# yangzhaojason/DualDiff

Measured on AMD Instinct MI355X. Metric: denoising-steps/sec, 6-view 224×400 fp16, 50-step DDIM @ 1/2/4/8 MI355X, higher is better.
Workload: dtype fp16; 1 GPU; BASELINE configs[1]: 6-view 224x400 (28x50 latents) multiview UNet + 2 ControlNet branches (ORS panorama + ORS-3D, SFA on), CFG 2.0 -> 12 view-instances/scene, DDIM-50 schedule, random-init weights; scenes_per_gpu=1, parallelism=scene-sharded x1 (no data-path collective), hip_graph=True, streams=3, invariant_conditioning=recomputed every step

## Files before the change

### dualdiff_amd/_native.py

```python
import ctypes
import os

import torch
from ctypes import (POINTER, Structure, c_char_p, c_float, c_int32, c_int64, c_uint32, c_void_p)

from . import _build

DD_F16, DD_BF16, DD_F32 = 0, 1, 2
DD_EPI_NONE, DD_EPI_GEGLU, DD_EPI_SILU = 0, 1, 2


class GemmDesc(Structure):
    _fields_ = [
        ("a", c_void_p), ("a2", c_void_p), ("lda", c_int64), ("lda2", c_int64), ("k1", c_int32),
        ("rows", c_int32), ("n", c_int32), ("k", c_int32),
        ("w", c_void_p), ("bias", c_void_p), ("rowvec", c_void_p),
        ("rows_per_inst", c_int32), ("ld_rowvec", c_int32),
        ("res", c_void_p), ("ldres", c_int64),
        ("out", c_void_p), ("ldc", c_int64),
        ("alpha", c_float), ("accumulate", c_int32), ("epilogue", c_int32),
        ("conv", c_int32), ("hin", c_int32), ("win", c_int32), ("cin", c_int32),
        ("hv", c_int32), ("wv", c_int32), ("hout", c_int32), ("wout", c_int32), ("stride", c_int32),
        ("dtype", c_int32), ("tile", c_int32), ("split_k", c_int32),
        ("ws", c_void_p), ("ws_bytes", c_int64),
# ... 28 lines not shown
        ("pos", c_void_p), ("cat", c_void_p), ("cls_out", c_void_p),
        ("rows", c_int32), ("points_per_box", c_int32), ("num_freqs", c_int32), ("include_input", c_int32),
        ("class_token_dim", c_int32), ("cls_offset", c_int32),
        ("ld_cat", c_int64),
        ("normalize", c_int32), ("points_dtype", c_int32), ("dtype", c_int32), ("n_classes", c_int32),
        ("freqs", c_float * 16), ("xyz_min", c_float * 3), ("xyz_range", c_float * 3),
    ]


class XAttnDesc(Structure):
    _fields_ = [
        ("x", c_void_p), ("ldx", c_int64), ("res", c_void_p), ("ldres", c_int64),
        ("wq", c_void_p), ("wo", c_void_p), ("bo", c_void_p),
        ("k", c_void_p), ("v", c_void_p), ("ldk", c_int64), ("ldv", c_int64),
        ("k_inst_stride", c_int64), ("k_head_stride", c_int64), ("v_inst_stride", c_int64), ("v_head_stride", c_int64),
        ("out", c_void_p), ("ldo", c_int64),
        ("instances", c_int32), ("rows_per_inst", c_int32), ("lk", c_int32),
        ("channels", c_int32), ("heads", c_int32), ("scale", c_float), ("dtype", c_int32),
        ("ln_out", c_void_p), ("ld_ln_out", c_int64), ("ln_gamma", c_void_p), ("ln_beta", c_void_p), ("ln_eps", c_float),
        ("lk_dev", c_void_p),
    ]


class Gemm8Desc(Structure):
    _fields_ = [
        ("a", c_void_p), ("a_scale", c_void_p), ("lda", c_int64),
        ("w", c_void_p), ("w_scale", c_void_p), ("ldw", c_int64),
        ("bias", c_void_p), ("res", c_void_p), ("ldres", c_int64),
        ("out", c_void_p), ("ldc", c_int64),
        ("rows", c_int32), ("n", c_int32), ("k_padded", c_int32), ("dtype", c_int32),
        ("out_headmajor_d", c_int32), ("hm_scaled_planes", c_int32), ("hm_scale", c_float), ("geglu", c_int32),
    ]


SIGNATURES = {
    "dd_abi_version": (c_int32, []),
    "dd_desc_size": (c_int64, [c_int32]),
    "dd_error_string": (c_char_p, [c_int32]),
    "dd_target_arch": (c_char_p, []),
    "dd_gemm": (c_int32, [POINTER(GemmDesc), c_void_p]),
    "dd_gemm_workspace_bytes": (c_int64, [POINTER(GemmDesc)]),
    "dd_gemm_num_tiles": (c_int32, []),
    "dd_gemm_tile_id": (c_int32, [c_int32]),
    "dd_gemm_kernel_name": (c_char_p, [POINTER(GemmDesc)]),
    "dd_gemm_conv_pad": (c_int32, [POINTER(GemmDesc), c_int32, c_void_p]),
    "dd_gemm_conv_pad_workspace_bytes": (c_int64, [POINTER(GemmDesc), c_int32]),
    "dd_gemm_conv_pad_kernel_name": (c_char_p, [POINTER(GemmDesc), c_int32]),
    "dd_groupnorm_nhwc": (c_int32, [c_void_p, c_int32, c_void_p, c_int32, c_void_p, c_void_p, c_void_p,
                                    c_int32, c_int32, c_int32, c_float, c_int32, c_int32,
                                    c_void_p, c_int64, c_void_p]),
    "dd_groupnorm_workspace_bytes": (c_int64, [c_int32, c_int32]),
    "dd_groupnorm_is_fused": (c_int32, [c_int32, c_int32, c_int32]),
    "dd_layernorm": (c_int32, [c_void_p, c_void_p, c_void_p, c_void_p, c_int64, c_int32, c_float,
                               c_int32, c_void_p]),
    "dd_attention": (c_int32, [POINTER(AttnDesc), c_void_p]),
    "dd_attention_kernel_name": (c_char_p, [POINTER(AttnDesc)]),
    "dd_add": (c_int32, [c_void_p, c_void_p, c_void_p, c_void_p, c_int64, c_int32, c_void_p]),
    "dd_scale": (c_int32, [c_void_p, c_void_p, c_float, c_int64, c_int32, c_void_p]),
    "dd_probe_spin": (c_int32, [c_void_p, c_uint32, c_void_p]),
    "dd_groupnorm_splitk": (c_int32, [c_void_p, c_int32, c_void_p, c_void_p, c_int32, c_void_p, c_int64, c_void_p,
                                      c_void_p, c_void_p, c_void_p, c_int32, c_int32, c_int32, c_int32, c_float, c_int32,
                                      c_int32, c_void_p]),
    "dd_xattn320": (c_int32, [POINTER(XAttnDesc), c_void_p]),
    "dd_nchw_to_nhwc_views": (c_int32, [c_void_p, c_void_p, c_int32, c_int32, c_int32, c_int32, c_int32, c_int32, c_int32,
                                        c_void_p]),
    "dd_fourier_embed_strided": (c_int32, [c_void_p, c_void_p, c_int64, c_int32, POINTER(c_float), c_int32, c_int32,
                                           c_int32, c_int32, c_int32, c_int64, c_int64, c_int64, c_int64, c_void_p]),
    "dd_box_tokens": (c_int32, [POINTER(BoxTokensDesc), c_void_p]),
    "dd_ctx_assemble": (c_int32, [c_void_p, c_void_p, c_void_p, c_void_p, c_void_p, c_int32, c_int32, c_int32, c_int32,
                                  c_int32, c_int32, c_int32, c_int32, c_void_p]),
    "dd_gemm8": (c_int32, [POINTER(Gemm8Desc), c_void_p]),
    "dd_rowquant_fp8": (c_int32, [c_void_p, c_void_p, c_void_p, c_void_p, c_void_p, c_int64, c_int32, c_int64, c_float,
                                  c_int32, c_void_p]),
    "dd_xattn_pack_weight": (c_int32, [c_void_p, c_void_p, c_int32, c_void_p]),
    "dd_silu": (c_int32, [c_void_p, c_void_p, c_int64, c_int32, c_void_p]),
    "dd_nchw_to_nhwc": (c_int32, [c_void_p, c_void_p, c_int32, c_int32, c_int32, c_int32, c_int32, c_void_p]),
    "dd_nhwc_to_nchw": (c_int32, [c_void_p, c_void_p, c_int32, c_int32, c_int32, c_int32, c_int32, c_void_p]),
    "dd_timestep_embedding": (c_int32, [c_void_p, c_void_p, c_int32, c_int32, c_int32, c_float,
                                        c_int32, c_void_p]),
    "dd_cfg_unipc_step": (c_int32, [c_void_p, c_void_p, c_void_p, c_void_p, c_void_p, c_void_p, c_void_p, c_void_p,
                                    c_float, c_int64, c_int32, c_void_p]),
    "dd_softmax_rows": (c_int32, [c_void_p, c_void_p, c_int64, c_int32, c_int64, c_int64, c_int32, c_void_p]),
    "dd_ors_project": (c_int32, [c_void_p, c_void_p, c_void_p, c_void_p, c_void_p, c_int32, c_int32, c_int32,
                                 c_float, c_int32, c_int32, c_int32, c_void_p]),
    "dd_fourier_embed": (c_int32, [c_void_p, c_void_p, c_int64, c_int32, POINTER(c_float), c_int32, c_int32,
                                   c_int32, c_int32, c_void_p]),
    "dd_conv3x3_small_cout": (c_int32, [c_void_p, c_void_p, c_void_p, c_void_p, c_int32, c_int32,
                                        c_int32, c_int32, c_int32, c_int32, c_void_p]),
    "dd_vae_posterior": (c_int32, [c_void_p, c_void_p, c_void_p, c_void_p, c_void_p, c_int32, c_int32, c_int32, c_float,
                                   c_int32, c_int32, c_void_p]),
# ... 70 lines not shown
```

### dualdiff_amd/csrc/elementwise.hip

```cpp
#include "dd_common.h"

namespace {

template <typename T>
__global__ __launch_bounds__(256)
void dd_add_kernel(const T* a, const T* b, const T* c, T* y, int64_t nvec) {
  for (int64_t i = (int64_t)blockIdx.x * blockDim.x + threadIdx.x; i < nvec;
       i += (int64_t)gridDim.x * blockDim.x) {
    float fa[8], fb[8];
    dd_unpack8<T>(dd_ld16(a + i * 8), fa);
    dd_unpack8<T>(dd_ld16(b + i * 8), fb);
#pragma unroll
    for (int e = 0; e < 8; ++e) fa[e] += fb[e];
    if (c) {
      dd_unpack8<T>(dd_ld16(c + i * 8), fb);
#pragma unroll
      for (int e = 0; e < 8; ++e) fa[e] += fb[e];
    }
    dd_st16(y + i * 8, dd_pack8<T>(fa));
  }
}

template <typename T, int OP>
__global__ __launch_bounds__(256)
void dd_unary_kernel(const T* x, T* y, float s, int64_t nvec) {
  for (int64_t i = (int64_t)blockIdx.x * blockDim.x + threadIdx.x; i < nvec;
       i += (int64_t)gridDim.x * blockDim.x) {
    float f[8];
    dd_unpack8<T>(dd_ld16(x + i * 8), f);
#pragma unroll
    for (int e = 0; e < 8; ++e) f[e] = OP == 0 ? f[e] * s : dd_silu_f(f[e]);
    dd_st16(y + i * 8, dd_pack8<T>(f));
  }
}

template <typename T>
__global__ __launch_bounds__(256)
void dd_nchw_to_nhwc_kernel(const T* x, T* y, int m, int c, int hw, int c_pad) {
  const int64_t total = (int64_t)m * hw * c_pad;
  for (int64_t i = (int64_t)blockIdx.x * blockDim.x + threadIdx.x; i < total;
       i += (int64_t)gridDim.x * blockDim.x) {
    const int ch = (int)(i % c_pad);
    const int64_t row = i / c_pad;
    const int px = (int)(row % hw);
    const int inst = (int)(row / hw);
    y[i] = ch < c ? x[((int64_t)inst * c + ch) * hw + px] : (T)0.f;
  }
}

template <typename T>
__global__ __launch_bounds__(256)
void dd_nhwc_to_nchw_kernel(const T* x, T* y, int m, int c, int hw, int ldx) {
// ... 207 lines not shown
  T* yout = y + (int64_t)inst * hout * wout * COUT;
#pragma unroll
  for (int rr = 0; rr < ROWS_PER_WAVE; ++rr) {
    const int oy = oy0 + wave * ROWS_PER_WAVE + rr;
    if (oy >= hout) continue;
    const int prow = (wave * ROWS_PER_WAVE + rr) * STRIDE;
#pragma unroll
    for (int g = 0; g < TW / 16; ++g) {
      const int ox = ox0 + g * 16 + px;
      if (ox0 + g * 16 >= wout) continue;
      const unsigned char* base = smem + (size_t)(prow * PW + (g * 16 + px) * STRIDE) * PIX;
      f32x4 acc[NB];
#pragma unroll
      for (int nb = 0; nb < NB; ++nb) acc[nb] = f32x4{0.f, 0.f, 0.f, 0.f};
#pragma unroll
      for (int ks = 0; ks < KSTEPS; ++ks) {
        const V8 xf = dd_as_v8<T>(*reinterpret_cast<const u32x4*>(base + koff[ks]));
#pragma unroll
        for (int nb = 0; nb < NB; ++nb) acc[nb] = dd_mfma16(wf[nb][ks], xf, acc[nb]);
      }
      if (ox < wout) {
#pragma unroll
        for (int nb = 0; nb < NB; ++nb) {
          V4 o;
#pragma unroll
          for (int r = 0; r < 4; ++r) {
            float v = acc[nb][r] + bv[nb][r];
            if (silu) v = dd_silu_f(v);
            o[r] = (T)v;
          }
          *reinterpret_cast<V4*>(yout + ((int64_t)oy * wout + ox) * COUT + nb * 16 + kc * 4) = o;
        }
      }
    }
  }
}

template <typename T>
__device__ __forceinline__ float dd_cfg_guided(const T* eps, int64_t i, int64_t n, float guidance) {
  const float eu = (float)eps[i], ec = (float)eps[n + i];
  return (float)(T)(eu + guidance * (ec - eu));
}

struct dd_ddim_coef {
  float sa_t, s1a_t, sa_p, s1a_p;
  __device__ explicit dd_ddim_coef(const float* c) : sa_t(c[0]), s1a_t(c[1]), sa_p(c[2]), s1a_p(c[3]) {}
  __device__ __forceinline__ float step(float xv, float e) const {
    const float x0 = (xv - s1a_t * e) / sa_t;
    return sa_p * x0 + s1a_p * e;
  }
  __device__ __forceinline__ float step(float xv, float e, float*, float*, float*, int64_t) const { return step(xv, e); }
};

struct dd_unipc_coef {
  float a_x, a_e, use_c, c_l, c_1, c_2, c_0, p_x, p_0, p_1;
  __device__ explicit dd_unipc_coef(const float* c)
      : a_x(c[0]), a_e(c[1]), use_c(c[2]), c_l(c[3]), c_1(c[4]), c_2(c[5]), c_0(c[6]), p_x(c[7]), p_0(c[8]),
        p_1(c[9]) {}
  __device__ __forceinline__ float step(float xv, float e, float* last, float* m1, float* m2, int64_t i) const {
    const float x0 = a_x * xv + a_e * e;
    const float o1 = m1[i];
    float xc = xv;
    if (use_c != 0.f) xc = c_l * last[i] + c_1 * o1 + c_2 * m2[i] + c_0 * x0;
    const float r = p_x * xc + p_0 * x0 + p_1 * o1;
    last[i] = xc;
    m2[i] = o1;
// ... 89 lines not shown
  for (int j = blockIdx.x * blockDim.x + threadIdx.x; j < view_elems; j += gridDim.x * blockDim.x) {
    const T r = dd_add_noise<T>(sa, s1a, clean[base + j], noise0[base + j]);
    x[base + j] = r;
    if (x_dup) x_dup[base + j] = r;
  }
}

inline unsigned grid_for(int64_t work, int per_block = 256, unsigned cap = 2048) {
  int64_t b = (work + per_block - 1) / per_block;
  if (b > cap) b = cap;
  if (b < 1) b = 1;
  return (unsigned)b;
}

}

extern "C" int dd_add(const void* a, const void* b, const void* c, void* y, int64_t n,
                      int32_t dtype, dd_stream_t stream) {
  if (!a || !b || !y || n <= 0 || (n & 7)) return DD_ERR_BAD_ARG;
  if (dtype != DD_F16 && dtype != DD_BF16) return DD_ERR_BAD_ARG;
  if (!dd_aligned16(a) || !dd_aligned16(b) || !dd_aligned16(y) || (c && !dd_aligned16(c))) return DD_ERR_BAD_ARG;
  hipStream_t s = reinterpret_cast<hipStream_t>(stream);
  dd_clear_error();
  const int64_t nvec = n / 8;
  if (dtype == DD_F16)
    hipLaunchKernelGGL(dd_add_kernel<_Float16>, dim3(grid_for(nvec)), dim3(256), 0, s,
                       (const _Float16*)a, (const _Float16*)b, (const _Float16*)c, (_Float16*)y, nvec);
  else
    hipLaunchKernelGGL(dd_add_kernel<__bf16>, dim3(grid_for(nvec)), dim3(256), 0, s,
                       (const __bf16*)a, (const __bf16*)b, (const __bf16*)c, (__bf16*)y, nvec);
  return dd_check_launch();
}

extern "C" int dd_scale(const void* x, void* y, float sc, int64_t n, int32_t dtype, dd_stream_t stream) {
  if (!x || !y || n <= 0 || (n & 7)) return DD_ERR_BAD_ARG;
  if (dtype != DD_F16 && dtype != DD_BF16) return DD_ERR_BAD_ARG;
  if (!dd_aligned16(x) || !dd_aligned16(y)) return DD_ERR_BAD_ARG;
  hipStream_t s = reinterpret_cast<hipStream_t>(stream);
  dd_clear_error();
  const int64_t nvec = n / 8;
  if (dtype == DD_F16)
    hipLaunchKernelGGL((dd_unary_kernel<_Float16, 0>), dim3(grid_for(nvec)), dim3(256), 0, s,
                       (const _Float16*)x, (_Float16*)y, sc, nvec);
  else
    hipLaunchKernelGGL((dd_unary_kernel<__bf16, 0>), dim3(grid_for(nvec)), dim3(256), 0, s,
                       (const __bf16*)x, (__bf16*)y, sc, nvec);
  return dd_check_launch();
}

extern "C" int dd_silu(const void* x, void* y, int64_t n, int32_t dtype, dd_stream_t stream) {
  if (!x || !y || n <= 0 || (n & 7)) return DD_ERR_BAD_ARG;
  if (dtype != DD_F16 && dtype != DD_BF16) return DD_ERR_BAD_ARG;
  if (!dd_aligned16(x) || !dd_aligned16(y)) return DD_ERR_BAD_ARG;
  hipStream_t s = reinterpret_cast<hipStream_t>(stream);
  dd_clear_error();
  const int64_t nvec = n / 8;
  if (dtype == DD_F16)
    hipLaunchKernelGGL((dd_unary_kernel<_Float16, 1>), dim3(grid_for(nvec)), dim3(256), 0, s,
                       (const _Float16*)x, (_Float16*)y, 1.f, nvec);
  else
    hipLaunchKernelGGL((dd_unary_kernel<__bf16, 1>), dim3(grid_for(nvec)), dim3(256), 0, s,
                       (const __bf16*)x, (__bf16*)y, 1.f, nvec);
  return dd_check_launch();
}

extern "C" int dd_nchw_to_nhwc(const void* x, void* y, int32_t m, int32_t c, int32_t hw,
// ... 77 lines not shown
  return dd_check_launch();
}

template <typename TI>
int launch_fourier(const void* x, void* out, int64_t total, int dims, const FourierFreqs& fr, int nf, int inc,
                   int out_dtype, hipStream_t s) {
  const unsigned g = (unsigned)grid_for(total > (1 << 30) ? (1 << 30) : (int)total);
  if (out_dtype == DD_F16)
    hipLaunchKernelGGL((dd_fourier_embed_kernel<TI, _Float16>), dim3(g), dim3(256), 0, s, (const TI*)x, (_Float16*)out, total, dims, fr, nf, inc);
  else if (out_dtype == DD_BF16)
    hipLaunchKernelGGL((dd_fourier_embed_kernel<TI, __bf16>), dim3(g), dim3(256), 0, s, (const TI*)x, (__bf16*)out, total, dims, fr, nf, inc);
  else
    hipLaunchKernelGGL((dd_fourier_embed_kernel<TI, float>), dim3(g), dim3(256), 0, s, (const TI*)x, (float*)out, total, dims, fr, nf, inc);
  return dd_check_launch();
}

extern "C" int dd_fourier_embed(const void* x, void* out, int64_t rows, int32_t dims, const float* freqs,
                                int32_t num_freqs, int32_t include_input, int32_t in_dtype, int32_t out_dtype,
                                dd_stream_t stream) {
  if (!x || !out || !freqs || rows <= 0 || dims <= 0) return DD_ERR_BAD_ARG;
  if (num_freqs <= 0 || num_freqs > 16) return DD_ERR_UNSUPPORTED;
  if (in_dtype < 0 || in_dtype > DD_F32 || out_dtype < 0 || out_dtype > DD_F32) return DD_ERR_BAD_ARG;
  FourierFreqs fr{};
  for (int i = 0; i < num_freqs; ++i) fr.f[i] = freqs[i];
  hipStream_t s = reinterpret_cast<hipStream_t>(stream);
  dd_clear_error();
  const int64_t total = rows * dims;
  const int inc = include_input ? 1 : 0;
  if (in_dtype == DD_F16) return launch_fourier<_Float16>(x, out, total, dims, fr, num_freqs, inc, out_dtype, s);
  if (in_dtype == DD_BF16) return launch_fourier<__bf16>(x, out, total, dims, fr, num_freqs, inc, out_dtype, s);
  return launch_fourier<float>(x, out, total, dims, fr, num_freqs, inc, out_dtype, s);
}

extern "C" int dd_conv3x3_small_cout(const void* x, const void* w, const void* bias, void* y_nchw,
                                     int32_t m, int32_t h, int32_t wd, int32_t cin, int32_t cout,
                                     int32_t dtype, dd_stream_t stream) {
  if (!x || !w || !y_nchw || m <= 0 || h <= 0 || wd <= 0 || cin <= 0 || cout <= 0) return DD_ERR_BAD_ARG;
  if ((cin & 7) || cout > 8) return DD_ERR_UNSUPPORTED;
  if (dtype != DD_F16 && dtype != DD_BF16) return DD_ERR_BAD_ARG;
  if (!dd_aligned16(x) || !dd_aligned16(w)) return DD_ERR_BAD_ARG;
  hipStream_t s = reinterpret_cast<hipStream_t>(stream);
  dd_clear_error();
  const int64_t npix = (int64_t)m * h * wd;
  const unsigned blocks = (unsigned)((npix + 3) / 4);
  if (dtype == DD_F16)
    hipLaunchKernelGGL((dd_conv3x3_small_kernel<_Float16, 8>), dim3(blocks), dim3(256), 0, s,
                       (const _Float16*)x, (const _Float16*)w, (const _Float16*)bias,
                       (_Float16*)y_nchw, m, h, wd, cin, cout);
  else
    hipLaunchKernelGGL((dd_conv3x3_small_kernel<__bf16, 8>), dim3(blocks), dim3(256), 0, s,
                       (const __bf16*)x, (const __bf16*)w, (const __bf16*)bias,
                       (__bf16*)y_nchw, m, h, wd, cin, cout);
  return dd_check_launch();
}

template <typename T, int CIN, int COUT, int STRIDE>
static int launch_thin(const void* x, const void* w, const void* bias, void* y, int m, int hin, int win, int hout, int wout,
                       int silu, hipStream_t s) {
  constexpr int TW = 64, TH = STRIDE == 1 ? 8 : 4;
  constexpr int PW = (TW - 1) * STRIDE + 3, PH = (TH - 1) * STRIDE + 3;
  constexpr int PIX = CIN * 2 + (CIN > 8 ? 16 : 0);
  constexpr size_t smem = (size_t)PH * PW * PIX;
  static_assert(smem <= 64 * 1024, "patch fits the default dynamic LDS limit");
  dim3 grid(((wout + TW - 1) / TW) * ((hout + TH - 1) / TH), m);
  hipLaunchKernelGGL((dd_conv3x3_thin_kernel<T, CIN, COUT, STRIDE>), grid, dim3(256), smem, s, (const T*)x, (const T*)w,
                     (const T*)bias, (T*)y, hin, win, hout, wout, silu);
  return dd_check_launch();
}

template <typename T>
static int launch_thin_t(const void* x, const void* w, const void* bias, void* y, int m, int hin, int win, int hout, int wout,
                         int cin, int cout, int stride, int silu, hipStream_t s) {
#define DD_THIN(CI, CO, ST) if (cin == CI && cout == CO && stride == ST) \
    return launch_thin<T, CI, CO, ST>(x, w, bias, y, m, hin, win, hout, wout, silu, s);
  DD_THIN(8, 16, 1) DD_THIN(16, 16, 1) DD_THIN(16, 32, 2) DD_THIN(32, 32, 1)
// ... 181 lines not shown
```

### dualdiff_amd/networks/unet_2d_condition_multiview.py

```python
from dataclasses import dataclass
from typing import Any, Dict, Optional, Tuple, Union

import torch
import torch.nn as nn

from .. import ops as O
from .blocks import BasicMultiviewTransformerBlock
from .layers import (BasicTransformerBlock, prefetch_cross_kv, drop_prefetched_kv, CrossKVBank, Conv3x3, CrossAttnDownBlock2D, CrossAttnUpBlock2D, DownBlock2D, GroupNorm,
                     TimestepEmbedding, Timesteps, UNetMidBlock2DCrossAttn, UpBlock2D, as_nchw_view,
                     run_down_block, run_up_block, to_nhwc, CTX_BASE, context_keys, ctx_capacity, lk_const)
from .model_base import ModelBase, sibling_overlap


def _at_capacity(ctx, cap):
    m, lc, c = ctx.shape
    if lc == cap:
        return ctx
    if ctx.stride(2) == 1 and ctx.stride(1) == c and ctx.stride(0) == cap * c and \
            (ctx.storage_offset() + m * cap * c) * ctx.element_size() <= ctx.untyped_storage().nbytes():
        return ctx.as_strided((m, cap, c), ctx.stride())
    buf = ctx.new_zeros((m, cap, c))
    buf[:, :lc] = ctx
    return buf


@dataclass
class UNet2DConditionOutput:
    sample: torch.Tensor


_DEFAULT_PAIR = {0: [5, 1], 1: [0, 2], 2: [1, 3], 3: [2, 4], 4: [3, 5], 5: [4, 0]}


class UNet2DConditionModelMultiview(ModelBase):
    multiview = True
    video = False
    prefetch_kv = __import__('os').environ.get('DD_PREFETCH_KV', '0') == '1'
    kv_bank = __import__('os').environ.get('DD_KV_BANK', '1') != '0'

    _WARN_ONCE = 0

    def __init__(
        self,
        sample_size: Optional[int] = None,
        in_channels: int = 4,
        out_channels: int = 4,
        center_input_sample: bool = False,
        flip_sin_to_cos: bool = True,
        freq_shift: int = 0,
        down_block_types: Tuple[str] = ("CrossAttnDownBlock2D", "CrossAttnDownBlock2D",
                                        "CrossAttnDownBlock2D", "DownBlock2D"),
        mid_block_type: Optional[str] = "UNetMidBlock2DCrossAttn",
        up_block_types: Tuple[str] = ("UpBlock2D", "CrossAttnUpBlock2D", "CrossAttnUpBlock2D",
                                      "CrossAttnUpBlock2D"),
        only_cross_attention: Union[bool, Tuple[bool]] = False,
        block_out_channels: Tuple[int] = (320, 640, 1280, 1280),
# ... 184 lines not shown
        with context_keys(ctx2d, lc, lk_dev):
            return [self.forward_nhwc(x, m, h, w, t_f32, ctx2d, lc, down_res, mid_res)]

    def forward_nhwc(self, x, m, h, w, t_f32, ctx2d, lc, down_res=None, mid_res=None):
        state = self.encode_nhwc(x, m, h, w, t_f32, ctx2d, lc)
        return self.decode_nhwc(state, down_res, mid_res)

    def encode_nhwc(self, x, m, h, w, t_f32, ctx2d, lc):
        dt = self.dtype
        if self.kv_bank:
            if self.__dict__.get("_kv_bank") is None:
                self.__dict__["_kv_bank"] = CrossKVBank(self)
            self.__dict__["_kv_bank"].run(ctx2d)
        elif self.prefetch_kv:
            if self.__dict__.get("_kv_stream") is None:
                self.__dict__["_kv_stream"] = torch.cuda.Stream()
            prefetch_cross_kv(self, ctx2d, self.__dict__["_kv_stream"])
        emb = self.time_embedding.run(self.time_proj.run(t_f32, dt))
        temb = self.temb_bank.run(O.silu(emb))
        forward_size = any(s % (2 ** self.num_upsamplers) != 0 for s in (h, w))
        x = self.conv_in.run(x, m, h, w)
        skips = [(x, h, w)]
        for blk in self.down_blocks:
            x, h, w, s = run_down_block(blk, x, m, h, w, temb, ctx2d, lc)
            skips += s
        x = self.mid_block.run(x, m, h, w, temb, ctx2d, lc)
        return {"x": x, "m": m, "h": h, "w": w, "skips": skips, "temb": temb, "ctx2d": ctx2d, "lc": lc,
                "forward_size": forward_size}

    def decode_nhwc(self, state, down_res=None, mid_res=None):
        x, m, h, w = state["x"], state["m"], state["h"], state["w"]
        skips, temb, ctx2d, lc = list(state["skips"]), state["temb"], state["ctx2d"], state["lc"]

        def plus(t, r):
            if not isinstance(r, (tuple, list)):
                r = (r,)
            if len(r) == 0:
                return t
            i = 0
            while i < len(r):
                t = O.add(t, r[i], r[i + 1]) if i + 1 < len(r) else O.add(t, r[i])
                i += 2
            return t

        if down_res is not None:
            if len(down_res) != len(skips):
                raise ValueError("expected %d down-block residuals, got %d" % (len(skips), len(down_res)))
            skips = [(plus(s, r), sh, sw) for (s, sh, sw), r in zip(skips, down_res)]
        if mid_res is not None:
            x = plus(x, mid_res)
        for i, blk in enumerate(self.up_blocks):
            final = i == len(self.up_blocks) - 1
            k = len(blk.resnets)
            up_size = None
            if not final:
                nxt = skips[-k - 1]
                up_size = (nxt[1], nxt[2]) if state["forward_size"] else None
            x, h, w = run_up_block(blk, x, m, h, w, skips, temb, ctx2d, lc, up_size)
        a = self.conv_norm_out.run(x, m, h * w, True)
        if self.__dict__.get("_kv_stream") is not None:
            drop_prefetched_kv(self, self.__dict__["_kv_stream"])
        if self.__dict__.get("_kv_bank") is not None:
            self.__dict__["_kv_bank"].drop()
        return O.conv3x3_small_cout(a, self.conv_out.packed, self.conv_out.bias, m, h, w)



class UNet2DConditionModel(UNet2DConditionModelMultiview):
    multiview = False



class UNet2DConditionModelMultiviewVideo(UNet2DConditionModelMultiview):
    video = True

    def set_n_frames(self, n_frames):
        from .video_blocks import VideoMultiviewTransformerBlock
        for mod in self.modules():
            if isinstance(mod, VideoMultiviewTransformerBlock):
                mod.n_frames = int(n_frames)
        self.config["n_frames"] = int(n_frames)

    def set_frame_shard(self, shard):
# ... 9 lines not shown
```

### dualdiff_amd/ops.py

```python
import collections as _collections
import ctypes
import os as _os

import torch

from . import _native, _timer, _workspace, tuning
from ._native import DD_BF16, DD_EPI_GEGLU, DD_EPI_NONE, DD_EPI_SILU, DD_F16, AttnDesc, Gemm8Desc, GemmDesc, XAttnDesc
from ._timer import KernelTimer, _stream, set_timer
from ._workspace import workspace, workspace_owner
from .tuning import (CHALLENGE_TILES, TUNE_TABLE_PATH, forget_tuned, load_tuned, save_tuned,
                     tune_candidates, tuned_table)

_THIN_CONV = _os.environ.get("DD_THIN_CONV", "1") != "0"
GN_SPLITK = _os.environ.get("DD_GN_SPLITK", "0") == "1"
LN_OUT_TILE = int(_os.environ.get("DD_LN_OUT_TILE", "0"))
XATTN_MAX_WGS = int(_os.environ.get("DD_XATTN_MAX_WGS", "256"))
CAUSAL_ATTN_MAX_L = 128
_ZERO_BIAS = {}
_FDT = {torch.float16: 0, torch.bfloat16: 1, torch.float32: 2}


def _dtype_code(dtype):
    if dtype == torch.float16:
        return DD_F16
    if dtype == torch.bfloat16:
        return DD_BF16
    raise TypeError("dualdiff_amd ops take fp16 / bf16 tensors, got %s" % dtype)


def _dt(t):
    return _dtype_code(t.dtype)


def _tname(code):
    return "f16" if code == DD_F16 else "bf16"


def _need_gpu(*ts):
    for t in ts:
        if t is not None and not t.is_cuda:
# ... 478 lines not shown
        bo = _ZERO_BIAS[key]
    d.bo = bo.data_ptr()
    d.k, d.ldk, d.k_inst_stride, d.k_head_stride = kv_operand(k)
    d.v, d.ldv, d.v_inst_stride, d.v_head_stride = kv_operand(v)
    d.out, d.ldo = out.data_ptr(), out.stride(0)
    d.instances, d.rows_per_inst, d.lk = int(instances), int(rows_per_inst), int(lk)
    d.channels, d.heads, d.scale, d.dtype = 320, 8, float(scale), _dt(x)
    d.lk_dev = lk_dev.data_ptr() if lk_dev is not None else None
    second = None
    if ln_out is not None:
        g_, b_, eps_ = ln_out
        _need_gpu(g_, b_)
        second = torch.empty((rows, 320), dtype=x.dtype, device=x.device)
        d.ln_out, d.ld_ln_out = second.data_ptr(), 320
        d.ln_gamma, d.ln_beta, d.ln_eps = g_.data_ptr(), b_.data_ptr(), float(eps_)
    _timer.launch("xattn320", lib.dd_xattn320, ctypes.byref(d), _stream(),
                  book=lambda: ("dd_xattn320_kernel", 4.0 * rows * 320 * 320 + 4.0 * rows * lk * 320,
                                2.0 * (rows * 320 * (2 + (1 if res is not None else 0) + (1 if second is not None else 0))
                                       + 2 * 320 * 320 + 2 * instances * lk * 320)))
    if second is not None:
        out._ln_out = second
    return out


def add(a, b, c=None, out=None):
    lib = _native.load()
    _need_gpu(a, b, c, out)
    out = _out_or_new(out, a, a.dtype, a.device, "add")
    _timer.launch("add", lib.dd_add, _ptr(a), _ptr(b), _ptr(c), _ptr(out), a.numel(), _dt(a), _stream(),
                  book=lambda: ("dd_add", 0.0, 2.0 * a.numel() * (3 + (1 if c is not None else 0))))
    return out


def scale(x, s, out=None):
    lib = _native.load()
    _need_gpu(x, out)
    out = _out_or_new(out, x, x.dtype, x.device, "scale")
    _native.check(lib.dd_scale(_ptr(x), _ptr(out), s, x.numel(), _dt(x), _stream()), "scale")
    return out


def silu(x, out=None):
    lib = _native.load()
    _need_gpu(x, out)
    out = _out_or_new(out, x, x.dtype, x.device, "silu")
    _native.check(lib.dd_silu(_ptr(x), _ptr(out), x.numel(), _dt(x), _stream()), "silu")
    return out


def nchw_to_nhwc(x, c_pad=None, views=1):
    lib = _native.load()
    _need_gpu(x)
    m, c, h, wt = x.shape
    if wt % views:
        raise ValueError("nchw_to_nhwc: width %d is not %d views" % (wt, views))
    c_pad = c if c_pad is None else c_pad
    x = x.contiguous()
    out = torch.empty((m * views * h * (wt // views), c_pad), dtype=x.dtype, device=x.device)
    if c_pad % 8 == 0:
        rc = lib.dd_nchw_to_nhwc_views(_ptr(x), _ptr(out), m, c, h, wt // views, views, c_pad, _dt(x), _stream())
    elif views == 1:
        rc = lib.dd_nchw_to_nhwc(_ptr(x), _ptr(out), m, c, h * wt, c_pad, _dt(x), _stream())
    else:
        raise ValueError("nchw_to_nhwc: a view split needs c_pad % 8 == 0")
    _native.check(rc, "nchw_to_nhwc")
    return out
# ... 330 lines not shown
```

### include/dualdiff_hip.h

```cpp
#ifndef DUALDIFF_HIP_H
#define DUALDIFF_HIP_H

#include <stdint.h>

#ifdef __cplusplus
extern "C" {
#endif

#define DD_ABI_VERSION 4

enum { DD_F16 = 0, DD_BF16 = 1 };

enum {
  DD_OK = 0,
  DD_ERR_BAD_ARG = -1,
  DD_ERR_UNSUPPORTED = -2,
  DD_ERR_LAUNCH = -3,
  DD_ERR_WORKSPACE = -4
};

typedef void* dd_stream_t;

int dd_abi_version(void);
int64_t dd_desc_size(int which);
// ... 79 lines not shown
  int32_t accumulate;
  int32_t dtype;
  int32_t variant;
  int64_t q_head_stride, k_head_stride, v_head_stride;
  int32_t q_prescaled;
  const int32_t* kv_batch_map2;
  const int32_t* lk_dev;
} dd_attn_desc;

int dd_attention(const dd_attn_desc* d, dd_stream_t stream);
const char* dd_attention_kernel_name(const dd_attn_desc* d);

typedef struct dd_xattn_desc {
  const void* x; int64_t ldx;
  const void* res; int64_t ldres;
  const void* wq; const void* wo; const void* bo;
  const void* k; const void* v; int64_t ldk, ldv;
  int64_t k_inst_stride, k_head_stride, v_inst_stride, v_head_stride;
  void* out; int64_t ldo;
  int32_t instances, rows_per_inst, lk;
  int32_t channels, heads;
  float scale;
  int32_t dtype;
  void* ln_out; int64_t ld_ln_out;
  const void* ln_gamma; const void* ln_beta; float ln_eps;
  const int32_t* lk_dev;
} dd_xattn_desc;

int dd_xattn320(const dd_xattn_desc* d, dd_stream_t stream);
int dd_xattn_pack_weight(const void* w, void* packed, int32_t dtype, dd_stream_t stream);

int dd_add(const void* a, const void* b, const void* c, void* y, int64_t n,
           int32_t dtype, dd_stream_t stream);
int dd_scale(const void* x, void* y, float s, int64_t n, int32_t dtype, dd_stream_t stream);
int dd_silu(const void* x, void* y, int64_t n, int32_t dtype, dd_stream_t stream);

int dd_nchw_to_nhwc(const void* x, void* y, int32_t m, int32_t c, int32_t hw,
                    int32_t c_pad, int32_t dtype, dd_stream_t stream);
int dd_nhwc_to_nchw(const void* x, void* y, int32_t m, int32_t c, int32_t hw,
                    int32_t ldx, int32_t dtype, dd_stream_t stream);

int dd_timestep_embedding(const float* t, void* out, int32_t n, int32_t dim,
                          int32_t flip_sin_to_cos, float freq_shift,
                          int32_t dtype, dd_stream_t stream);

#define DD_F32 2
int dd_fourier_embed(const void* x, void* out, int64_t rows, int32_t dims, const float* freqs,
                     int32_t num_freqs, int32_t include_input, int32_t in_dtype, int32_t out_dtype,
                     dd_stream_t stream);

int dd_nchw_to_nhwc_views(const void* x, void* y, int32_t m, int32_t c, int32_t h, int32_t w, int32_t views,
                          int32_t c_pad, int32_t dtype, dd_stream_t stream);
int dd_fourier_embed_strided(const void* x, void* out, int64_t rows, int32_t dims, const float* freqs,
                             int32_t num_freqs, int32_t include_input, int32_t in_dtype, int32_t out_dtype,
                             int32_t inner, int64_t stride_outer, int64_t stride_inner, int64_t stride_dim,
                             int64_t out_ld, dd_stream_t stream);
typedef struct dd_box_tokens_desc {
  const void* points; const int64_t* classes; const uint8_t* masks;
  const void* class_tokens; const void* null_pos; const void* null_class;
  void* pos; void* cat; void* cls_out;
  int32_t rows, points_per_box, num_freqs, include_input, class_token_dim, cls_offset;
  int64_t ld_cat;
  int32_t normalize, points_dtype, dtype;
  int32_t n_classes;
  float freqs[16]; float xyz_min[3]; float xyz_range[3];
} dd_box_tokens_desc;
// ... 85 lines not shown
```

Before: 94.36 steps/s.

## Batch ControlNet residual adds into one multi-tensor launch and tile small-cout conv

Replaces the per-skip chain of elementwise add launches for the ControlNet down/mid residuals with a grouped add_multi kernel. One launch covers up to 16 tensors, with blocks partitioned across items by a prefix table. It also adds a new LDS-tiled, double-buffered MFMA 3x3 conv for small output-channel counts (the conv_out path) that reuses the input halo and weights from shared memory. The aim is to cut launch overhead and redundant global loads, at the cost of more code paths and tile shapes chosen by heuristic.

```diff
diff --git a/dualdiff_amd/_native.py b/dualdiff_amd/_native.py
--- a/dualdiff_amd/_native.py
+++ b/dualdiff_amd/_native.py
@@ -84,6 +84,12 @@
         ("out_headmajor_d", c_int32), ("hm_scaled_planes", c_int32), ("hm_scale", c_float), ("geglu", c_int32),
     ]
 
+
+class AddItem(Structure):
+    _fields_ = [("a", c_void_p), ("b", c_void_p), ("c", c_void_p), ("y", c_void_p), ("n", c_int64)]
+
+
+ADD_MULTI_MAX = 16
 
 SIGNATURES = {
     "dd_abi_version": (c_int32, []),
@@ -108,6 +114,7 @@
     "dd_attention": (c_int32, [POINTER(AttnDesc), c_void_p]),
     "dd_attention_kernel_name": (c_char_p, [POINTER(AttnDesc)]),
     "dd_add": (c_int32, [c_void_p, c_void_p, c_void_p, c_void_p, c_int64, c_int32, c_void_p]),
+    "dd_add_multi": (c_int32, [POINTER(AddItem), c_int32, c_int32, c_void_p]),
     "dd_scale": (c_int32, [c_void_p, c_void_p, c_float, c_int64, c_int32, c_void_p]),
     "dd_probe_spin": (c_int32, [c_void_p, c_uint32, c_void_p]),
     "dd_groupnorm_splitk": (c_int32, [c_void_p, c_int32, c_void_p, c_void_p, c_int32, c_void_p, c_int64, c_void_p,
diff --git a/dualdiff_amd/csrc/elementwise.hip b/dualdiff_amd/csrc/elementwise.hip
--- a/dualdiff_amd/csrc/elementwise.hip
+++ b/dualdiff_amd/csrc/elementwise.hip
@@ -18,6 +18,62 @@
       for (int e = 0; e < 8; ++e) fa[e] += fb[e];
     }
     dd_st16(y + i * 8, dd_pack8<T>(fa));
+  }
+}
+
+constexpr int ADD_MULTI_VPT = 4;
+constexpr int ADD_MULTI_VPB = 256 * ADD_MULTI_VPT;
+constexpr int64_t ADD_MULTI_MAX_BLOCKS = 4096;
+
+struct dd_add_multi_args {
+  dd_add_item item[DD_ADD_MULTI_MAX];
+  uint32_t end[DD_ADD_MULTI_MAX];
+  int32_t count;
+};
+
+template <typename T>
+__global__ __launch_bounds__(256)
+void dd_add_multi_kernel(const dd_add_multi_args args) {
+  int it = 0;
+#pragma unroll
+  for (int i = 0; i < DD_ADD_MULTI_MAX - 1; ++i)
+    if (i + 1 < args.count && blockIdx.x >= args.end[i]) it = i + 1;
+  const uint32_t first = it ? args.end[it - 1] : 0u;
+  const int64_t nblk = args.end[it] - first;
+  const T* a = (const T*)args.item[it].a;
+  const T* b = (const T*)args.item[it].b;
+  const T* c = (const T*)args.item[it].c;
+  T* y = (T*)args.item[it].y;
+  const int64_t nvec = args.item[it].n;
+  for (int64_t base = (int64_t)(blockIdx.x - first) * ADD_MULTI_VPB + threadIdx.x; base < nvec;
+       base += nblk * ADD_MULTI_VPB) {
+    u32x4 va[ADD_MULTI_VPT], vb[ADD_MULTI_VPT], vc[ADD_MULTI_VPT];
+#pragma unroll
+    for (int j = 0; j < ADD_MULTI_VPT; ++j) {
+      const int64_t i = base + j * 256;
+      if (i < nvec) {
+        va[j] = dd_ld16(a + i * 8);
+        vb[j] = dd_ld16(b + i * 8);
+        if (c) vc[j] = dd_ld16(c + i * 8);
+      }
+    }
+#pragma unroll
+    for (int j = 0; j < ADD_MULTI_VPT; ++j) {
+      const int64_t i = base + j * 256;
+      if (i < nvec) {
+        float fa[8], fb[8];
+        dd_unpack8<T>(va[j], fa);
+        dd_unpack8<T>(vb[j], fb);
+#pragma unroll
+        for (int e = 0; e < 8; ++e) fa[e] += fb[e];
+        if (c) {
+          dd_unpack8<T>(vc[j], fb);
+#pragma unroll
+          for (int e = 0; e < 8; ++e) fa[e] += fb[e];
+        }
+        dd_st16(y + i * 8, dd_pack8<T>(fa));
+      }
+    }
   }
 }
 
@@ -291,6 +347,133 @@
           *reinterpret_cast<V4*>(yout + ((int64_t)oy * wout + ox) * COUT + nb * 16 + kc * 4) = o;
         }
       }
+    }
+  }
+}
+
+template <int TH, int TW, int CK>
+struct dd_conv_cout8_cfg {
+  static constexpr int PW = TW + 2, PH = TH + 2;
+  static constexpr int PIX = CK * 2 + 16;
+  static constexpr int VPP = CK / 8;
+  static constexpr int NVEC = PH * PW * VPP;
+  static constexpr int NLD = (NVEC + 255) / 256;
+  static constexpr int WROW = 9 * CK * 2 + 16;
+  static constexpr int WVEC = 8 * 9 * VPP;
+  static constexpr int WLD = (WVEC + 255) / 256;
+  static constexpr int PBUF = PH * PW * PIX, WBUF = 8 * WROW;
+  static constexpr int LDS = 2 * (PBUF + WBUF);
+  static constexpr int GROUPS = TW / 16, UNITS = TH * GROUPS, UPW = UNITS / 4;
+  static_assert(TW % 16 == 0 && UNITS % 4 == 0 && CK % 32 == 0, "tile shape");
+  static_assert(LDS <= 64 * 1024, "static LDS limit; two workgroups per CU need <= 80 KB");
+};
+
+template <typename T, int TH, int TW, int CK>
+__global__ __launch_bounds__(256)
+void dd_conv3x3_cout8_kernel(const T* __restrict__ x, const T* __restrict__ w, const T* __restrict__ bias,
+                             T* __restrict__ y, int h, int wd, int cin, int cout) {
+  using C = dd_conv_cout8_cfg<TH, TW, CK>;
+  using V8 = typename dd_vec<T>::v8;
+  __shared__ __attribute__((aligned(16))) unsigned char smem[C::LDS];
+
+  const int tid = threadIdx.x, lane = tid & 63;
+  const int wave = __builtin_amdgcn_readfirstlane(tid >> 6);
+  const int px = lane & 15, kc = lane >> 4;
+  const int tiles_x = (wd + TW - 1) / TW;
+  const int ty = blockIdx.x / tiles_x, tx = blockIdx.x - ty * tiles_x;
+  const int inst = blockIdx.y;
+  const int oy0 = ty * TH, ox0 = tx * TW;
+  const T* xin = x + (int64_t)inst * h * wd * cin;
+  const int nchunks = cin / CK;
+
+  u32x4 pv[C::NLD], wv[C::WLD];
+  auto load_chunk = [&](int ch) {
+    const int c0 = ch * CK;
+#pragma unroll
+    for (int i = 0; i < C::NLD; ++i) {
+      const int v = tid + i * 256;
+      const int pix = v / C::VPP, cv = v - pix * C::VPP;
+      const int py = pix / C::PW, pxx = pix - py * C::PW;
+      const int iy = oy0 - 1 + py, ix = ox0 - 1 + pxx;
+      pv[i] = u32x4{0u, 0u, 0u, 0u};
+      if (v < C::NVEC && iy >= 0 && iy < h && ix >= 0 && ix < wd)
+        pv[i] = dd_ld16(xin + ((int64_t)iy * wd + ix) * cin + c0 + cv * 8);
+    }
+#pragma unroll
+    for (int i = 0; i < C::WLD; ++i) {
+      const int v = tid + i * 256;
+      const int row = v / (9 * C::VPP), r = v - row * (9 * C::VPP);
+      const int tap = r / C::VPP, cv = r - tap * C::VPP;
+      wv[i] = u32x4{0u, 0u, 0u, 0u};
+      if (row < cout) wv[i] = dd_ld16(w + ((int64_t)row * 9 + tap) * cin + c0 + cv * 8);
+    }
+  };
+  auto store_chunk = [&](int b) {
+    unsigned char* pb = smem + b * C::PBUF;
+    unsigned char* wb = smem + 2 * C::PBUF + b * C::WBUF;
+#pragma unroll
+    for (int i = 0; i < C::NLD; ++i) {
+      const int v = tid + i * 256;
+      const int pix = v / C::VPP, cv = v - pix * C::VPP;
+      if (v < C::NVEC) *reinterpret_cast<u32x4*>(pb + pix * C::PIX + cv * 16) = pv[i];
+    }
+#pragma unroll
+    for (int i = 0; i < C::WLD; ++i) {
+      const int v = tid + i * 256;
+      const int row = v / (9 * C::VPP), r = v - row * (9 * C::VPP);
+      if (row < cout) *reinterpret_cast<u32x4*>(wb + row * C::WROW + r * 16) = wv[i];
+    }
+  };
+
+  f32x4 acc[C::UPW];
+#pragma unroll
+  for (int u = 0; u < C::UPW; ++u) acc[u] = f32x4{0.f, 0.f, 0.f, 0.f};
+  const bool wrow = px < cout;
+  const int wlane = (wrow ? px : 0) * C::WROW + kc * 16;
+  const int xlane = px * C::PIX + kc * 16;
+
+  load_chunk(0);
+  store_chunk(0);
+  __syncthreads();
+  for (int ch = 0; ch < nchunks; ++ch) {
+    const bool more = ch + 1 < nchunks;
+    if (more) load_chunk(ch + 1);
+    const unsigned char* pb = smem + (ch & 1) * C::PBUF + xlane;
+    const unsigned char* wb = smem + 2 * C::PBUF + (ch & 1) * C::WBUF + wlane;
+#pragma unroll
+    for (int tap = 0; tap < 9; ++tap) {
+#pragma unroll
+      for (int ks = 0; ks < CK / 32; ++ks) {
+        u32x4 wraw = *reinterpret_cast<const u32x4*>(wb + tap * CK * 2 + ks * 64);
+        if (!wrow) wraw = u32x4{0u, 0u, 0u, 0u};
+        const V8 wf = dd_as_v8<T>(wraw);
+#pragma unroll
+        for (int u = 0; u < C::UPW; ++u) {
+          const int unit = wave * C::UPW + u;
+          const int ry = unit / C::GROUPS, g = unit - ry * C::GROUPS;
+          const V8 xf = dd_as_v8<T>(*reinterpret_cast<const u32x4*>(
+              pb + ((ry + tap / 3) * C::PW + g * 16 + tap % 3) * C::PIX + ks * 64));
+          acc[u] = dd_mfma16(xf, wf, acc[u]);
+        }
+      }
+    }
+    if (more) store_chunk((ch + 1) & 1);
+    __syncthreads();
+  }
+
+  if (!wrow) return;
+  const float bv = bias ? (float)bias[px] : 0.f;
+  T* yout = y + ((int64_t)inst * cout + px) * h * wd;
+#pragma unroll
+  for (int u = 0; u < C::UPW; ++u) {
+    const int unit = wave * C::UPW + u;
+    const int ry = unit / C::GROUPS, g = unit - ry * C::GROUPS;
+    const int oy = oy0 + ry;
+    if (oy >= h) continue;
+#pragma unroll
+    for (int r = 0; r < 4; ++r) {
+      const int ox = ox0 + g * 16 + kc * 4 + r;
+      if (ox < wd) yout[(int64_t)oy * wd + ox] = (T)(acc[u][r] + bv);
     }
   }
 }
@@ -446,6 +629,39 @@
   return dd_check_launch();
 }
 
+extern "C" int dd_add_multi(const dd_add_item* items, int32_t count, int32_t dtype, dd_stream_t stream) {
+  if (!items || count < 1 || count > DD_ADD_MULTI_MAX) return DD_ERR_BAD_ARG;
+  if (dtype != DD_F16 && dtype != DD_BF16) return DD_ERR_BAD_ARG;
+  int order[DD_ADD_MULTI_MAX];
+  for (int i = 0; i < count; ++i) {
+    const dd_add_item& t = items[i];
+    if (!t.a || !t.b || !t.y || t.n <= 0 || (t.n & 7)) return DD_ERR_BAD_ARG;
+    if (!dd_aligned16(t.a) || !dd_aligned16(t.b) || !dd_aligned16(t.y) || (t.c && !dd_aligned16(t.c))) return DD_ERR_BAD_ARG;
+    int j = i;
+    for (; j > 0 && items[order[j - 1]].n < t.n; --j) order[j] = order[j - 1];
+    order[j] = i;
+  }
+  dd_add_multi_args args{};
+  args.count = count;
+  uint32_t total = 0;
+  for (int i = 0; i < count; ++i) {
+    args.item[i] = items[order[i]];
+    const int64_t nvec = args.item[i].n / 8;
+    args.item[i].n = nvec;
+    int64_t blocks = (nvec + ADD_MULTI_VPB - 1) / ADD_MULTI_VPB;
+    if (blocks > ADD_MULTI_MAX_BLOCKS) blocks = ADD_MULTI_MAX_BLOCKS;
+    total += (uint32_t)blocks;
+    args.end[i] = total;
+  }
+  hipStream_t s = reinterpret_cast<hipStream_t>(stream);
+  dd_clear_error();
+  if (dtype == DD_F16)
+    hipLaunchKernelGGL(dd_add_multi_kernel<_Float16>, dim3(total), dim3(256), 0, s, args);
+  else
+    hipLaunchKernelGGL(dd_add_multi_kernel<__bf16>, dim3(total), dim3(256), 0, s, args);
+  return dd_check_launch();
+}
+
 extern "C" int dd_scale(const void* x, void* y, float sc, int64_t n, int32_t dtype, dd_stream_t stream) {
   if (!x || !y || n <= 0 || (n & 7)) return DD_ERR_BAD_ARG;
   if (dtype != DD_F16 && dtype != DD_BF16) return DD_ERR_BAD_ARG;
@@ -589,6 +805,22 @@
   return launch_fourier<float>(x, out, total, dims, fr, num_freqs, inc, out_dtype, s);
 }
 
+template <typename T, int TH, int TW, int CK>
+static void launch_cout8(const void* x, const void* w, const void* bias, void* y, int m, int h, int wd, int cin, int cout,
+                         hipStream_t s) {
+  dim3 grid(((wd + TW - 1) / TW) * ((h + TH - 1) / TH), m);
+  hipLaunchKernelGGL((dd_conv3x3_cout8_kernel<T, TH, TW, CK>), grid, dim3(256), 0, s, (const T*)x, (const T*)w,
+                     (const T*)bias, (T*)y, h, wd, cin, cout);
+}
+
+template <typename T>
+static void launch_cout8_t(const void* x, const void* w, const void* bias, void* y, int m, int h, int wd, int cin, int cout,
+                           hipStream_t s) {
+  if ((int64_t)m * h * wd >= 65536) launch_cout8<T, 8, 32, 32>(x, w, bias, y, m, h, wd, cin, cout, s);
+  else if (cin % 64 == 0) launch_cout8<T, 4, 16, 64>(x, w, bias, y, m, h, wd, cin, cout, s);
+  else launch_cout8<T, 4, 16, 32>(x, w, bias, y, m, h, wd, cin, cout, s);
+}
+
 extern "C" int dd_conv3x3_small_cout(const void* x, const void* w, const void* bias, void* y_nchw,
                                      int32_t m, int32_t h, int32_t wd, int32_t cin, int32_t cout,
                                      int32_t dtype, dd_stream_t stream) {
@@ -598,6 +830,11 @@
   if (!dd_aligned16(x) || !dd_aligned16(w)) return DD_ERR_BAD_ARG;
   hipStream_t s = reinterpret_cast<hipStream_t>(stream);
   dd_clear_error();
+  if (cin % 32 == 0 && m <= 65535) {
+    if (dtype == DD_F16) launch_cout8_t<_Float16>(x, w, bias, y_nchw, m, h, wd, cin, cout, s);
+    else launch_cout8_t<__bf16>(x, w, bias, y_nchw, m, h, wd, cin, cout, s);
+    return dd_check_launch();
+  }
   const int64_t npix = (int64_t)m * h * wd;
   const unsigned blocks = (unsigned)((npix + 3) / 4);
   if (dtype == DD_F16)
diff --git a/dualdiff_amd/networks/unet_2d_condition_multiview.py b/dualdiff_amd/networks/unet_2d_condition_multiview.py
--- a/dualdiff_amd/networks/unet_2d_condition_multiview.py
+++ b/dualdiff_amd/networks/unet_2d_condition_multiview.py
@@ -22,6 +22,22 @@
     buf = ctx.new_zeros((m, cap, c))
     buf[:, :lc] = ctx
     return buf
+
+
+def residual_sums(targets, residuals):
+    res = [tuple(r) if isinstance(r, (tuple, list)) else (r,) for r in residuals]
+    out = list(targets)
+    k = 0
+    while True:
+        live = [j for j, r in enumerate(res) if len(r) > 2 * k]
+        if not live:
+            return out
+        for g in range(0, len(live), O.ADD_MULTI_MAX):
+            group = live[g:g + O.ADD_MULTI_MAX]
+            sums = O.add_multi([(out[j],) + res[j][2 * k:2 * k + 2] for j in group])
+            for j, s in zip(group, sums):
+                out[j] = s
+        k += 1
 
 
 @dataclass
@@ -272,23 +288,13 @@
         x, m, h, w = state["x"], state["m"], state["h"], state["w"]
         skips, temb, ctx2d, lc = list(state["skips"]), state["temb"], state["ctx2d"], state["lc"]
 
-        def plus(t, r):
-            if not isinstance(r, (tuple, list)):
-                r = (r,)
-            if len(r) == 0:
-                return t
-            i = 0
-            while i < len(r):
-                t = O.add(t, r[i], r[i + 1]) if i + 1 < len(r) else O.add(t, r[i])
-                i += 2
-            return t
-
-        if down_res is not None:
-            if len(down_res) != len(skips):
-                raise ValueError("expected %d down-block residuals, got %d" % (len(skips), len(down_res)))
-            skips = [(plus(s, r), sh, sw) for (s, sh, sw), r in zip(skips, down_res)]
-        if mid_res is not None:
-            x = plus(x, mid_res)
+        if down_res is not None and len(down_res) != len(skips):
+            raise ValueError("expected %d down-block residuals, got %d" % (len(skips), len(down_res)))
+        targets = [s for s, _, _ in skips] + [x]
+        res = (list(down_res) if down_res is not None else [()] * len(skips)) + [mid_res if mid_res is not None else ()]
+        targets = residual_sums(targets, res)
+        skips = [(t, sh, sw) for t, (_, sh, sw) in zip(targets, skips)]
+        x = targets[-1]
         for i, blk in enumerate(self.up_blocks):
             final = i == len(self.up_blocks) - 1
             k = len(blk.resnets)
diff --git a/dualdiff_amd/ops.py b/dualdiff_amd/ops.py
--- a/dualdiff_amd/ops.py
+++ b/dualdiff_amd/ops.py
@@ -5,7 +5,7 @@
 import torch
 
 from . import _native, _timer, _workspace, tuning
-from ._native import DD_BF16, DD_EPI_GEGLU, DD_EPI_NONE, DD_EPI_SILU, DD_F16, AttnDesc, Gemm8Desc, GemmDesc, XAttnDesc
+from ._native import ADD_MULTI_MAX, DD_BF16, DD_EPI_GEGLU, DD_EPI_NONE, DD_EPI_SILU, DD_F16, AttnDesc, Gemm8Desc, GemmDesc, XAttnDesc
 from ._timer import KernelTimer, _stream, set_timer
 from ._workspace import workspace, workspace_owner
 from .tuning import (CHALLENGE_TILES, TUNE_TABLE_PATH, forget_tuned, load_tuned, save_tuned,
@@ -550,6 +550,29 @@
     return out
 
 
+def add_multi(items, outs=None):
+    lib = _native.load()
+    items = [tuple(it) + (None,) * (3 - len(it)) for it in items]
+    if not 1 <= len(items) <= ADD_MULTI_MAX:
+        raise ValueError("add_multi: %d items, 1 .. %d fit one launch" % (len(items), ADD_MULTI_MAX))
+    outs = [None] * len(items) if outs is None else list(outs)
+    if len(outs) != len(items):
+        raise ValueError("add_multi: %d outputs for %d items" % (len(outs), len(items)))
+    table = (_native.AddItem * len(items))()
+    nbytes = 0.0
+    for i, (a, b, c) in enumerate(items):
+        _need_gpu(a, b, c, outs[i])
+        if a.dtype != items[0][0].dtype:
+            raise TypeError("add_multi: one dtype per launch")
+        outs[i] = _out_or_new(outs[i], a, a.dtype, a.device, "add_multi")
+        t = table[i]
+        t.a, t.b, t.c, t.y, t.n = a.data_ptr(), b.data_ptr(), None if c is None else c.data_ptr(), outs[i].data_ptr(), a.numel()
+        nbytes += 2.0 * a.numel() * (3 + (1 if c is not None else 0))
+    _timer.launch("add_multi", lib.dd_add_multi, table, len(items), _dt(items[0][0]), _stream(),
+                  book=lambda: ("dd_add_multi", 0.0, nbytes))
+    return outs
+
+
 def scale(x, s, out=None):
     lib = _native.load()
     _need_gpu(x, out)
diff --git a/include/dualdiff_hip.h b/include/dualdiff_hip.h
--- a/include/dualdiff_hip.h
+++ b/include/dualdiff_hip.h
@@ -135,6 +135,12 @@
 
 int dd_add(const void* a, const void* b, const void* c, void* y, int64_t n,
            int32_t dtype, dd_stream_t stream);
+#define DD_ADD_MULTI_MAX 16
+typedef struct dd_add_item {
+  const void* a; const void* b; const void* c; void* y;
+  int64_t n;
+} dd_add_item;
+int dd_add_multi(const dd_add_item* items, int32_t count, int32_t dtype, dd_stream_t stream);
 int dd_scale(const void* x, void* y, float s, int64_t n, int32_t dtype, dd_stream_t stream);
 int dd_silu(const void* x, void* y, int64_t n, int32_t dtype, dd_stream_t stream);
 
```

New measurement: 95.08 steps/s, median of 6. Within noise of the previous version (+0.8%).
